# romanwerpachowski/ML

Measured on NVIDIA B200. Metric: em_point_components_per_second, higher is better.
Workload: dtype f64

## Files before the change

### ml_b200/csrc/em.cu

```cuda
#include <algorithm>
#include <cmath>
#include <limits>

#include "em_direct.cuh"
#include "em_split.cuh"
#include "fastmath.cuh"
#include "internal.h"

namespace mlb {

constexpr int kTile = 64;
constexpr int kEmThreads = 128;
constexpr int kLogBatch = 16;

__host__ __device__ constexpr int em_ne_offdiag(int DP) { return 4 * (DP / 4) * (DP / 4 - 1) / 2; }
__host__ __device__ constexpr int em_ne(int DP) { return em_ne_offdiag(DP) + 2 * (DP / 4) + (DP / 4 + 1) / 2 + DP / 4; }
__host__ __device__ constexpr int em_estep_offdiag(int DP, int a, int mb)
{
    const int DQ = DP / 4, ma = a / 4, i = a % 4;
    int n = 0;
    for (int m = 0; m < ma; ++m) n += 4 * (DQ - 1 - m);
    return n + i * (DQ - 1 - ma) + (mb - ma - 1);
}
__host__ __device__ constexpr int em_fm_raw(int DP) { return 1 + DP + DP * (DP + 1) / 2; }
__host__ __device__ constexpr int em_nm(int DP) { return (em_fm_raw(DP) + 7) / 8; }
__host__ __device__ constexpr int em_sv(int DP, int KP) { return em_nm(DP) * 8 * KP + 8; }
__host__ __device__ constexpr int em_theta_len(int DP, int KP) { return em_ne(DP) * (KP / 8) * 32 + KP; }

constexpr size_t em_smem_bytes(int DP, int KP)
{
    return sizeof(double) * (em_theta_len(DP, KP) + 2 * kTile * (DP + 4) + kTile * (KP + 4) + 8 + DP + kExpTableSize);
}

struct EmArgs {
    const double* x;
    long long n_local;
    int d, k;
    const double* shift;
    const double* theta;
    const int2* feat_m;
    double* partials;
    int chunk;
    int n_chunks;
    unsigned* counter;
    const double* r_in;
    long long r_ld;
    double* r_out;
    long long r_out_ld;
    unsigned* labels_out;
    long long range_begin, range_count;
};

__device__ __forceinline__ long long min64(long long a, long long b) { return a < b ? a : b; }

__device__ __forceinline__ void dmma(double (&acc)[2], double a, double b)
{
    asm("mma.sync.aligned.m8n8k4.row.col.f64.f64.f64.f64 {%0,%1}, {%2}, {%3}, {%0,%1};" : "+d"(acc[0]), "+d"(acc[1]) : "d"(a), "d"(b));
}

template <int NT>
__device__ __forceinline__ void load_theta_frag(const double* thE, int j, int lane, double (&bf)[NT])
{
    if constexpr (NT == 1) {
        bf[0] = thE[j * 32 + lane];
    } else {
#pragma unroll
        for (int h = 0; h < NT / 2; ++h) {
            const double2 v = reinterpret_cast<const double2*>(thE)[(j * (NT / 2) + h) * 32 + lane];
            bf[2 * h] = v.x;
            bf[2 * h + 1] = v.y;
        }
    }
}

template <int DP, int KP, int MODE>
__global__ void __launch_bounds__(kEmThreads, (DP * KP <= 128 || MODE >= 2) ? 4 : 2) em_kernel(const EmArgs p)
{
    constexpr int NT = KP / 8, DQ = DP / 4, NE = em_ne(DP), NM = em_nm(DP);
    constexpr int ZS = DP + 4, RS = KP + 4;
    constexpr int WN = (NM >= 8 || NT == 1) ? 1 : 2, WM = 4 / WN;
    constexpr int MW = (NM + WM - 1) / WM, NW = NT / WN;
    constexpr int SV = em_sv(DP, KP);
    constexpr int XR = kTile * DP / kEmThreads;

    extern __shared__ __align__(16) double sm[];
    double* thE = sm;
    double* cE = thE + NE * NT * 32;
    double* Zb = cE + KP;
    double* R = Zb + 2 * kTile * ZS;
    double* wl = R + kTile * RS;
    double* sh = wl + 8;
    double* etab = sh + DP;
    __shared__ int s_next;

    const int tid = threadIdx.x, lane = tid & 31, warp = tid >> 5, g = lane >> 2, c = lane & 3;
    const int d = p.d;

    if (MODE != 1)
        for (int i = tid; i < em_theta_len(DP, KP); i += kEmThreads) sm[i] = p.theta[i];
    for (int i = tid; i < 2 * kTile * ZS; i += kEmThreads) Zb[i] = 0.0;
    for (int i = tid; i < kTile * RS; i += kEmThreads) R[i] = 0.0;
    if (tid < DP) sh[tid] = tid < d ? p.shift[tid] : 0.0;
    load_exp_table(etab);

    const int wm = warp / WN, wn = warp % WN;
    int ia[MW], ib[MW];
    double sacc[MW][NW][2];
    if (MODE < 2) {
#pragma unroll
        for (int i = 0; i < MW; ++i) {
            const int mt = wm * MW + i;
            const int2 f = mt < NM ? p.feat_m[mt * 8 + g] : make_int2(DP + 1, DP + 1);
            ia[i] = f.x;
            ib[i] = f.y;
        }
    }

    double xr[XR];
    auto load_tile = [&](long long point0, int nvalid) {
        const double* xg = p.x + point0 * d;
        const int nel = nvalid * d;
#pragma unroll
        for (int r = 0; r < XR; ++r) {
            const int e = tid + kEmThreads * r;
            xr[r] = e < nel ? xg[e] : 0.0;
        }
    };
    auto store_tile = [&](double* Z, int nvalid) {
        const int nel = nvalid * d;
#pragma unroll
        for (int r = 0; r < XR; ++r) {
            const int e = tid + kEmThreads * r;
            if (e < kTile * d) {
                const int pt = (d == DP) ? e / DP : FastDiv(d).div(e);
                const int dm = e - pt * d;
                Z[pt * ZS + dm] = e < nel ? xr[r] - sh[dm] : 0.0;
            }
        }
        if (tid < kTile) Z[tid * ZS + DP] = tid < nvalid ? 1.0 : 0.0;
    };

    const long long work_begin = MODE >= 2 ? p.range_begin : 0;
    const long long work_end = MODE >= 2 ? p.range_begin + p.range_count : p.n_local;

    for (;;) {
        __syncthreads();
        if (tid == 0) s_next = static_cast<int>(atomicAdd(p.counter, 1u));
        __syncthreads();
        const int chunk = s_next;
        if (chunk >= p.n_chunks) break;
        const long long p_begin = work_begin + static_cast<long long>(chunk) * p.chunk;
        const long long p_end = min64(p_begin + p.chunk, work_end);
        const int ntiles = static_cast<int>((p_end - p_begin + kTile - 1) / kTile);

        if (MODE < 2) {
#pragma unroll
            for (int i = 0; i < MW; ++i)
#pragma unroll
                for (int nt = 0; nt < NW; ++nt) sacc[i][nt][0] = sacc[i][nt][1] = 0.0;
        }
        double ll_acc = 0.0, ll_prod = 1.0;

        load_tile(p_begin, static_cast<int>(min64(kTile, p_end - p_begin)));
        store_tile(Zb, static_cast<int>(min64(kTile, p_end - p_begin)));
        __syncthreads();

        for (int t = 0; t < ntiles; ++t) {
            double* Z = Zb + (t & 1) * kTile * ZS;
            const long long tile0 = p_begin + static_cast<long long>(t) * kTile;
            const int nvalid = static_cast<int>(min64(kTile, p_end - tile0));
            const int nvalid_next = t + 1 < ntiles ? static_cast<int>(min64(kTile, p_end - tile0 - kTile)) : 0;
            if (t + 1 < ntiles) load_tile(tile0 + kTile, nvalid_next);

            if (MODE == 1) {
                for (int idx = tid; idx < kTile * p.k; idx += kEmThreads) {
                    const int pt = idx % kTile, kk = idx / kTile;
                    R[pt * RS + kk] = pt < nvalid ? p.r_in[tile0 + pt + kk * p.r_ld] : 0.0;
                }
            } else {
                const double* z0 = Z + (warp * 16 + g) * ZS;
                const double* z1 = z0 + 8 * ZS;
                double acc[2][NT][2];
#pragma unroll
                for (int nt = 0; nt < NT; ++nt) {
                    const double2 cc = *reinterpret_cast<const double2*>(cE + 8 * nt + 2 * c);
                    acc[0][nt][0] = acc[1][nt][0] = cc.x;
                    acc[0][nt][1] = acc[1][nt][1] = cc.y;
                }
                double zc0[DQ], zc1[DQ];
#pragma unroll
                for (int m = 0; m < DQ; ++m) {
                    zc0[m] = z0[4 * m + c];
                    zc1[m] = z1[4 * m + c];
                }
                auto estep = [&](int j, double a0, double a1) {
                    double bf[NT];
                    load_theta_frag<NT>(thE, j, lane, bf);
#pragma unroll
                    for (int nt = 0; nt < NT; ++nt) {
                        dmma(acc[0][nt], a0, bf[nt]);
                        dmma(acc[1][nt], a1, bf[nt]);
                    }
                };
#pragma unroll
                for (int a = 0; a < DP - 4; ++a) {
                    const double za0 = z0[a], za1 = z1[a];
#pragma unroll
                    for (int m = a / 4 + 1; m < DQ; ++m) estep(em_estep_offdiag(DP, a, m), za0 * zc0[m], za1 * zc1[m]);
                }
                constexpr int J0 = em_ne_offdiag(DP);
#pragma unroll
                for (int m = 0; m < DQ; ++m) estep(J0 + m, zc0[m] * zc0[m], zc1[m] * zc1[m]);
#pragma unroll
                for (int m = 0; m < DQ; ++m) {
                    const int o = 4 * m + ((c + 1) & 3);
                    estep(J0 + DQ + m, zc0[m] * z0[o], zc1[m] * z1[o]);
                }
#pragma unroll
                for (int h = 0; h < (DQ + 1) / 2; ++h) {
                    const int mx = 2 * h + (c >> 1);
                    const int o = 4 * mx + c, o2 = 4 * mx + ((c + 2) & 3);
                    const bool live = mx < DQ;
                    const double u0 = live ? z0[o] * z0[o2] : 0.0, u1 = live ? z1[o] * z1[o2] : 0.0;
                    estep(J0 + 2 * DQ + h, u0, u1);
                }
#pragma unroll
                for (int m = 0; m < DQ; ++m) estep(NE - DQ + m, zc0[m], zc1[m]);
                double mxs[2], sums[2];
#pragma unroll
                for (int mt = 0; mt < 2; ++mt) {
                    int mkey = lse_key(acc[mt][0][0]);
#pragma unroll
                    for (int nt = 0; nt < NT; ++nt) mkey = max(mkey, max(lse_key(acc[mt][nt][0]), lse_key(acc[mt][nt][1])));
                    mkey = max(mkey, __shfl_xor_sync(0xffffffffu, mkey, 1));
                    mkey = max(mkey, __shfl_xor_sync(0xffffffffu, mkey, 2));
                    const double mx = lse_shift_of_key(mkey);
                    double sum = 0.0;
#pragma unroll
                    for (int nt = 0; nt < NT; ++nt) {
                        acc[mt][nt][0] = exp_nonpositive(acc[mt][nt][0] - mx, etab);
                        acc[mt][nt][1] = exp_nonpositive(acc[mt][nt][1] - mx, etab);
                        sum += acc[mt][nt][0] + acc[mt][nt][1];
                    }
                    sum += __shfl_xor_sync(0xffffffffu, sum, 1);
                    sum += __shfl_xor_sync(0xffffffffu, sum, 2);
                    mxs[mt] = mx;
                    sums[mt] = sum;
                }
                const double inv_mine = reciprocal_of_sum((c & 1) ? sums[1] : sums[0]);
                const double invs[2] = {__shfl_sync(0xffffffffu, inv_mine, lane & ~1), __shfl_sync(0xffffffffu, inv_mine, lane | 1)};
#pragma unroll
                for (int mt = 0; mt < 2; ++mt) {
                    const int pl = warp * 16 + mt * 8 + g;
                    const double inv = invs[mt];
                    if (c == 0 && pl < nvalid) {
                        ll_acc += mxs[mt];
                        ll_prod *= sums[mt];
                    }
                    if (MODE == 0) {
#pragma unroll
                        for (int nt = 0; nt < NT; ++nt)
                            *reinterpret_cast<double2*>(R + pl * RS + 8 * nt + 2 * c) = make_double2(acc[mt][nt][0] * inv, acc[mt][nt][1] * inv);
                    } else if (MODE == 3) {
                        if (c == 0 && pl < nvalid) p.r_out[(tile0 - p.range_begin) + pl] = (mxs[mt] + log(sums[mt])) - 0.5 * d * kLog2Pi;
                    } else {
                        double best = -1.0;
                        unsigned best_k = 0xffffffffu;
#pragma unroll
                        for (int nt = 0; nt < NT; ++nt)
#pragma unroll
                            for (int e = 0; e < 2; ++e) {
                                const int kk = 8 * nt + 2 * c + e;
                                const double r = acc[mt][nt][e] * inv;
                                if (kk < p.k) {
                                    if (pl < nvalid && p.r_out) p.r_out[(tile0 - p.range_begin) + pl + kk * p.r_out_ld] = r;
                                    if (r > best) { best = r; best_k = kk; }
                                }
                            }
#pragma unroll
                        for (int off = 1; off <= 2; off <<= 1) {
                            const double ob = __shfl_xor_sync(0xffffffffu, best, off);
                            const unsigned ok = __shfl_xor_sync(0xffffffffu, best_k, off);
                            if (ob > best || (ob == best && ok < best_k)) { best = ob; best_k = ok; }
                        }
                        if (c == 0 && pl < nvalid && p.labels_out) p.labels_out[(tile0 - p.range_begin) + pl] = best_k;
                    }
                }
            }
            if (MODE < 2) {
                __syncthreads();
#pragma unroll 4
                for (int s = 0; s < kTile / 4; ++s) {
                    const double* zp = Z + (4 * s + c) * ZS;
                    const double* rp = R + (4 * s + c) * RS + wn * NW * 8 + g;
                    double bf[NW];
#pragma unroll
                    for (int nt = 0; nt < NW; ++nt) bf[nt] = rp[8 * nt];
#pragma unroll
                    for (int i = 0; i < MW; ++i) {
                        if (wm * MW + i < NM) {
                            const double af = zp[ia[i]] * zp[ib[i]];
#pragma unroll
                            for (int nt = 0; nt < NW; ++nt) dmma(sacc[i][nt], af, bf[nt]);
                        }
                    }
                }
            }
            if (MODE != 1 && ((t & (kLogBatch - 1)) == kLogBatch - 1 || t + 1 == ntiles)) {
                ll_acc += log(ll_prod);
                ll_prod = 1.0;
            }
            if (t + 1 < ntiles) store_tile(Zb + ((t + 1) & 1) * kTile * ZS, nvalid_next);
            __syncthreads();
        }

        if (MODE < 2) {
            double* out = p.partials + static_cast<long long>(chunk) * SV;
#pragma unroll
            for (int i = 0; i < MW; ++i) {
                const int mt = wm * MW + i;
                if (mt < NM) {
#pragma unroll
                    for (int nt = 0; nt < NW; ++nt)
                        *reinterpret_cast<double2*>(out + (mt * 8 + g) * KP + (wn * NW + nt) * 8 + 2 * c) = make_double2(sacc[i][nt][0], sacc[i][nt][1]);
                }
            }
#pragma unroll
            for (int off = 16; off >= 1; off >>= 1) ll_acc += __shfl_xor_sync(0xffffffffu, ll_acc, off);
            if (lane == 0) wl[warp] = ll_acc;
            __syncthreads();
            if (tid == 0) out[NM * 8 * KP] = (wl[0] + wl[1]) + (wl[2] + wl[3]);
            if (tid >= 1 && tid < 8) out[NM * 8 * KP + tid] = 0.0;
        }
    }
}

#include "em_small.cuh"

struct EmFinalizeArgs {
    const double* vsum;
    const double* dstats;
    const double* shift;
    int d, k, DP, KP, SV;
    int DPd, dSV;
    long long n_total;
    const int2* feat_m;
    const int2* feat_e;
    int nm8, ne;
    double* means;
    double* covs;
    double* weights;
    double* inv_covs;
    double* sqrt_dets;
    double* theta_out;
    double* dimg_out;
    double* kappa_out;
    int p_in_smem;
    double* ll_ring;
    unsigned long long* ll_counter;
    int ll_ring_len;
};

__global__ void em_finalize_kernel(const EmFinalizeArgs p)
{
    extern __shared__ double fs[];
// ... 220 lines not shown
    double* ll_tile = nullptr;
    double* partials = nullptr;
    double* vsum = nullptr;
    long long* sc_begin = nullptr;
    int2* tile_tab = nullptr;
    int n_sc = 0;
    int grid_e = 0, grid_m = 0;
};

struct EmDirect {
    bool capable = false;
    bool ready = false;
    int DP = 0, NB = 0, KPr = 0, IMG = 0, L = 0, SVd = 0;
    int cb = 1, cg = 1, tiles_per_range = 0, n_ranges = 1;
    size_t smem_e = 0, smem_m = 0;
    int64_t sc_bounds[kVirtualShards + 1] = {};
    std::vector<EmDirectGpu> gpus;
    ReduceScratch scratch;
};

constexpr int kDirectMaxDim = 128;
constexpr double kKappaDirect = 3.0e5;

constexpr int kLlRing = 4096;
constexpr long long kStagePoints = 1 << 20;

}

using namespace mlb;

struct mlb_em {
    mlb_ctx* ctx = nullptr;
    mlb_data* data = nullptr;
    int d = 0, k = 0, DP = 0, KP = 0, NT = 0, NE = 0, NM = 0, SV = 0;
    std::vector<int2> feat_m, feat_e;
    std::vector<EmGpu> gpus;
    int cur = 0;
    bool have_params = false, have_step = false;
    int last_path = 0;
    int64_t direct_steps = 0;
    int64_t launches = 0;
    int64_t steps_done = 0;
    EmKernelFn fn_step = nullptr, fn_mstep = nullptr, fn_emit = nullptr, fn_score = nullptr;
    int path = 1;
    EmDirect dr;
    int forced_path = 0;
    int route = 1;
    double kappa_max = 0.0;
    bool r_direct_valid = false;
    double* kappa_host = nullptr;
    EmSplitKernelFn fn_split_e = nullptr, fn_split_m = nullptr, fn_split_score = nullptr;
    size_t smem_split_e = 0, smem_split_m = 0;
    size_t smem_fused = 0;
    int MW = 4;
    cudaGraphExec_t step_graph[2] = {nullptr, nullptr};
    int64_t launches_per_step = 0;
    int plain_steps = 0;
    ReduceScratch reduce_scratch;

    double* means(int g) const { return gpus[g].params; }
    double* covs(int g) const { return gpus[g].params + d * k; }
    double* weights(int g) const { return covs(g) + static_cast<size_t>(k) * d * d; }
    double* inv_covs(int g) const { return weights(g) + k; }
    double* sqrt_dets(int g) const { return inv_covs(g) + static_cast<size_t>(k) * d * d; }
    size_t params_len() const { return static_cast<size_t>(d) * k + 2 * static_cast<size_t>(k) * d * d + 2 * k; }
};

namespace mlb {

static int pad_to(int v, const int* options, int n)
{
    for (int i = 0; i < n; ++i)
        if (v <= options[i]) return options[i];
    return 0;
}

static EmArgs base_args(const mlb_em* em, int g)
{
    const DataShard& sh = em->data->shards[g];
    const EmGpu& eg = em->gpus[g];
    EmArgs a{};
    a.x = sh.x;
    a.n_local = sh.n();
    a.d = em->d;
    a.k = em->k;
    a.shift = sh.shift;
    a.theta = eg.theta[em->cur];
    a.feat_m = eg.feat_m;
    a.partials = eg.partials;
    a.chunk = em->data->lay.chunk;
    a.n_chunks = static_cast<int>(sh.n_chunks());
    a.counter = eg.counter;
    return a;
}

static int launch_em(mlb_em* em, EmKernelFn fn, const EmArgs& a, int g, int grid)
{
    Gpu& gpu = em->ctx->gpus[g];
    MLB_CUDA(cudaMemsetAsync(a.counter, 0, sizeof(unsigned), gpu.stream));
    if (a.n_chunks > 0) {
        const bool timed = fn == em->fn_step;
        if (timed) MLB_TRY(em->gpus[g].timer.begin(gpu.stream));
        fn<<<std::min(grid, a.n_chunks), em->DP <= 8 ? kSmallThreads : kEmThreads, em->smem_fused, gpu.stream>>>(a);
        MLB_CUDA(cudaGetLastError());
        if (timed) MLB_TRY(em->gpus[g].timer.end(gpu.stream));
        ++em->launches;
    }
    return MLB_OK;
}

static EmSplitArgs split_args(const mlb_em* em, int g, const double* theta)
{
    const DataShard& sh = em->data->shards[g];
    const EmGpu& eg = em->gpus[g];
    EmSplitArgs a{};
    a.x = sh.x;
    a.n_local = sh.n();
    a.d = em->d; a.k = em->k; a.DP = em->DP; a.KP = em->KP;
    a.shift = sh.shift;
    a.theta = theta;
    a.feat_e = eg.feat_e_off;
    a.feat_m = eg.feat_m;
    a.ne = em->NE; a.nm = em->NM;
    a.r = eg.r;
    a.partials = eg.partials;
    a.ll_tile = eg.ll_tile;
    a.sv = em->SV;
    a.chunk = em->data->lay.chunk;
    a.n_chunks = static_cast<int>(sh.n_chunks());
    a.counter = eg.counter;
    return a;
}

static int launch_split(mlb_em* em, int g, const double* theta, bool run_e, bool timed)
{
    Gpu& gpu = em->ctx->gpus[g];
    EmGpu& eg = em->gpus[g];
    const EmSplitArgs a = split_args(em, g, theta);
    if (a.n_chunks == 0) return MLB_OK;
    if (timed) MLB_TRY(eg.timer.begin(gpu.stream));
    if (run_e) {
        MLB_CUDA(cudaMemsetAsync(a.counter, 0, sizeof(unsigned), gpu.stream));
        const long long e_items = static_cast<long long>(a.n_chunks) * (a.chunk / kSpTile);
        em->fn_split_e<<<static_cast<unsigned>(std::min<long long>(eg.grid_e, e_items)), kSpThreads, em->smem_split_e, gpu.stream>>>(a);
        MLB_CUDA(cudaGetLastError());
        ++em->launches;
    }
    const int ngroups = em->KP / (em->NT * 8), nslabs = (em->NM + 4 * em->MW - 1) / (4 * em->MW);
    const long long nitems = static_cast<long long>(a.n_chunks) * nslabs * ngroups;
    MLB_REQUIRE(nitems < (1ll << 31), "EM split path: too many work items");
    MLB_CUDA(cudaMemsetAsync(a.counter, 0, sizeof(unsigned), gpu.stream));
    em->fn_split_m<<<static_cast<unsigned>(std::min<long long>(eg.grid_m, nitems)), kSpThreads, em->smem_split_m, gpu.stream>>>(a);
    MLB_CUDA(cudaGetLastError());
    ++em->launches;
    if (timed) MLB_TRY(eg.timer.end(gpu.stream));
    return MLB_OK;
// ... 505 lines not shown

extern "C" {

int mlb_selftest_exp(const double* x, int64_t n, double* out)
{
    MLB_REQUIRE(x && out && n >= 0, "mlb_selftest_exp: bad argument");
    if (n == 0) return MLB_OK;
    MLB_CUDA(cudaSetDevice(0));
    double *dx = nullptr, *dy = nullptr;
    MLB_CUDA(cudaMalloc(&dx, sizeof(double) * n));
    MLB_CUDA(cudaMalloc(&dy, sizeof(double) * n));
    MLB_CUDA(cudaMemcpy(dx, x, sizeof(double) * n, cudaMemcpyHostToDevice));
    selftest_exp_kernel<<<static_cast<unsigned>((n + 127) / 128), 128>>>(dx, n, dy);
    MLB_CUDA(cudaGetLastError());
    MLB_CUDA(cudaMemcpy(out, dy, sizeof(double) * n, cudaMemcpyDeviceToHost));
    MLB_CUDA(cudaFree(dx));
    MLB_CUDA(cudaFree(dy));
    return MLB_OK;
}

int mlb_em_create(mlb_ctx* ctx, mlb_data* data, int k, mlb_em** out)
{
    MLB_ENTER(ctx);
    MLB_REQUIRE(ctx && data && out, "mlb_em_create: null argument");
    MLB_REQUIRE(data->ctx == ctx, "mlb_em_create: data belongs to another context");
    MLB_REQUIRE(k >= 1, "mlb_em_create: number of components must be positive");
    MLB_REQUIRE(data->d <= kDirectMaxDim, "mlb_em_create: D=%d not supported by this build (D <= %d)", data->d, kDirectMaxDim);
    static const int dps[] = {4, 8, 16}, kps[] = {8, 16, 32};
    const bool fused = data->d <= 16 && k <= 32;
    const bool split = !fused && data->d <= 64 && k <= 256;
    int DP = 0, KP = 0, NT = 0;
    if (fused) {
        DP = pad_to(data->d, dps, 3);
        KP = pad_to(k, kps, 3);
        NT = KP / 8;
    } else if (split) {
        DP = (data->d + 3) / 4 * 4;
        const int KG = k > 32 ? 64 : (k > 16 ? 32 : 16);
        KP = (k + KG - 1) / KG * KG;
        NT = KG / 8;
    }
    auto* em = new mlb_em;
    em->ctx = ctx; em->data = data; em->d = data->d; em->k = k;
    em->path = fused ? 1 : split ? 2 : 0;
    em->route = em->path ? em->path : 3;
    if (em->path) {
        em->DP = DP; em->KP = KP; em->NT = NT; em->NE = em_ne(DP); em->NM = em_nm(DP); em->SV = em_sv(DP, KP);
    }
    if (fused) {
        em->fn_step = em_kernel_for<0>(DP, KP);
        em->fn_mstep = em_kernel_for<1>(DP, KP);
        em->fn_emit = em_kernel_for<2>(DP, KP);
        em->fn_score = em_kernel_for<3>(DP, KP);
        em->smem_fused = DP <= 8 ? em_small_smem_bytes(DP, KP) : em_smem_bytes(DP, KP);
    } else if (split) {
        em->fn_split_e = NT == 8 ? em_split_e_kernel<8> : NT == 4 ? em_split_e_kernel<4> : em_split_e_kernel<2>;
        em->fn_split_score = NT == 8 ? em_split_e_kernel<8 + kSpScore> : NT == 4 ? em_split_e_kernel<4 + kSpScore> : em_split_e_kernel<2 + kSpScore>;
        int best_waste = 1 << 30;
        for (int mw = 3; mw <= 5; ++mw) {
            const int slabs = (em->NM + 4 * mw - 1) / (4 * mw), waste = slabs * 4 * mw - em->NM;
            if (waste <= best_waste) { best_waste = waste; em->MW = mw; }
        }
        if (NT == 8) em->fn_split_m = em->MW == 3 ? em_split_m_kernel<8, 3> : em->MW == 4 ? em_split_m_kernel<8, 4> : em_split_m_kernel<8, 5>;
        else if (NT == 4) em->fn_split_m = em->MW == 3 ? em_split_m_kernel<4, 3> : em->MW == 4 ? em_split_m_kernel<4, 4> : em_split_m_kernel<4, 5>;
        else em->fn_split_m = em->MW == 3 ? em_split_m_kernel<2, 3> : em->MW == 4 ? em_split_m_kernel<2, 4> : em_split_m_kernel<2, 5>;
        em->smem_split_e = em_split_e_smem(NT, DP, KP);
        em->smem_split_m = em_split_m_smem(NT, DP);
    }
    if (em->path) {
        em->feat_e.assign(static_cast<size_t>(em->NE) * 4, make_int2(-1, -1));
        const int DQ = DP / 4, J0 = em_ne_offdiag(DP);
        auto put = [&](int j, int c, int a, int b) { em->feat_e[static_cast<size_t>(j) * 4 + c] = make_int2(std::min(a, b), std::max(a, b)); };
        for (int a = 0; a < DP - 4; ++a)
            for (int m = a / 4 + 1; m < DQ; ++m)
                for (int c = 0; c < 4; ++c) put(em_estep_offdiag(DP, a, m), c, a, 4 * m + c);
        for (int m = 0; m < DQ; ++m)
            for (int c = 0; c < 4; ++c) {
                put(J0 + m, c, 4 * m + c, 4 * m + c);
                put(J0 + DQ + m, c, 4 * m + c, 4 * m + ((c + 1) & 3));
            }
        for (int h = 0; h < (DQ + 1) / 2; ++h)
            for (int c = 0; c < 4; ++c) {
                const int mx = 2 * h + (c >> 1);
                if (mx < DQ) put(J0 + 2 * DQ + h, c, 4 * mx + c, 4 * mx + ((c + 2) & 3));
            }
        for (int m = 0; m < DQ; ++m)
            for (int c = 0; c < 4; ++c) em->feat_e[static_cast<size_t>(em->NE - DQ + m) * 4 + c] = make_int2(4 * m + c, DP);
        em->feat_m.assign(static_cast<size_t>(em->NM) * 8, make_int2(DP + 1, DP + 1));
        size_t f = 0;
        em->feat_m[f++] = make_int2(DP, DP);
        for (int a = 0; a < DP; ++a) em->feat_m[f++] = make_int2(a, DP);
        for (int a = 0; a < DP; ++a)
            for (int b = a; b < DP; ++b) em->feat_m[f++] = make_int2(a, b);
    }
    if (fused && DP <= 8) {
        for (size_t f = 0; f < em->feat_m.size(); ++f) {
            int2 ab = make_int2(DP + 1, DP + 1);
            if (f < em->feat_e.size() && em->feat_e[f].x >= 0) ab = em->feat_e[f];
            if (static_cast<int>(f) == em_small_count_slot(DP)) ab = make_int2(DP, DP);
            em->feat_m[f] = ab;
        }
    }
    {
        EmDirect& dr = em->dr;
        dr.capable = true;
        dr.DP = (em->d + 7) / 8 * 8;
        dr.NB = dr.DP / 8;
        dr.KPr = (k + 7) / 8 * 8;
        dr.IMG = dr_img_len(dr.DP);
        dr.L = dr_stat_len(dr.DP);
        const long long svd = static_cast<long long>(k) * dr.L + 8;
        if (svd >= (1ll << 31)) { delete em; set_error("mlb_em_create: D=%d, K=%d: statistics vector too long", data->d, k); return MLB_EINVAL; }
        dr.SVd = static_cast<int>(svd);
        dr.cb = static_cast<int>(std::max<size_t>(1, std::min<size_t>(std::min(16, k), (12 * 1024) / (sizeof(double) * dr.IMG))));
        const int T = dr_tiles(dr.NB);
        if (T <= 4 * kDrSlots) {
            const int by_smem = static_cast<int>((96 * 1024) / (sizeof(double) * 2 * kDrSub * (dr.DP + 12))) - 1;
            dr.cg = std::max(1, std::min({16, k, 4 * kDrSlots / T, by_smem}));
            dr.tiles_per_range = T;
            dr.n_ranges = 1;
        } else {
            dr.cg = 1;
            dr.tiles_per_range = 4 * kDrSlots;
            dr.n_ranges = (T + 4 * kDrSlots - 1) / (4 * kDrSlots);
        }
        dr.smem_e = em_direct_e_smem(dr.DP, dr.cb);
        dr.smem_m = em_direct_m_smem(dr.DP, dr.cg, em->d);
        dr.sc_bounds[0] = 0;
        for (int v = 0; v < kVirtualShards; ++v)
            dr.sc_bounds[v + 1] = dr.sc_bounds[v] + std::min<int64_t>(data->lay.vshard_chunk[v + 1] - data->lay.vshard_chunk[v], kDrSuperPerVshard);
        dr.gpus.resize(ctx->gpus.size());
    }
    em->gpus.resize(ctx->gpus.size());
    int rc = for_each_gpu(ctx, [&](int g, Gpu& gpu) -> int {
        EmGpu& eg = em->gpus[g];
        EmDirectGpu& dg = em->dr.gpus[g];
        const DataShard& sh = data->shards[g];
        MLB_CUDA(cudaMallocFromPoolAsync(&eg.params, sizeof(double) * em->params_len(), gpu.pool, gpu.stream));
        MLB_CUDA(cudaMallocFromPoolAsync(&eg.ll, sizeof(double) * kLlRing, gpu.pool, gpu.stream));
        MLB_CUDA(cudaMallocFromPoolAsync(&eg.ll_counter, sizeof(unsigned long long), gpu.pool, gpu.stream));
        MLB_CUDA(cudaMemsetAsync(eg.ll_counter, 0, sizeof(unsigned long long), gpu.stream));
        MLB_CUDA(cudaMallocFromPoolAsync(&eg.counter, sizeof(unsigned), gpu.pool, gpu.stream));
        MLB_CUDA(cudaMallocFromPoolAsync(&dg.img, sizeof(double) * static_cast<size_t>(k) * em->dr.IMG, gpu.pool, gpu.stream));
        MLB_CUDA(cudaMallocFromPoolAsync(&dg.kappa, sizeof(double) * k, gpu.pool, gpu.stream));
        MLB_CUDA(cudaMemsetAsync(dg.kappa, 0, sizeof(double) * k, gpu.stream));
        {
            const size_t fin_smem = finalize_smem(em, nullptr);
            if (fin_smem > 48 * 1024)
                MLB_CUDA(cudaFuncSetAttribute(reinterpret_cast<const void*>(em_finalize_kernel), cudaFuncAttributeMaxDynamicSharedMemorySize, static_cast<int>(fin_smem)));
        }
        int sms = 0;
        MLB_CUDA(cudaDeviceGetAttribute(&sms, cudaDevAttrMultiProcessorCount, gpu.device));
        if (em->path) {
            const size_t theta_len = static_cast<size_t>(em_theta_len(DP, KP));
            MLB_CUDA(cudaMallocFromPoolAsync(&eg.theta[0], sizeof(double) * theta_len, gpu.pool, gpu.stream));
            MLB_CUDA(cudaMallocFromPoolAsync(&eg.theta[1], sizeof(double) * theta_len, gpu.pool, gpu.stream));
            MLB_CUDA(cudaMallocFromPoolAsync(&eg.partials, sizeof(double) * std::max<int64_t>(1, sh.n_chunks()) * em->SV, gpu.pool, gpu.stream));
            MLB_CUDA(cudaMallocFromPoolAsync(&eg.vsum, sizeof(double) * kVirtualShards * em->SV, gpu.pool, gpu.stream));
            MLB_CUDA(cudaMallocFromPoolAsync(&eg.feat_m, sizeof(int2) * em->feat_m.size(), gpu.pool, gpu.stream));
            MLB_CUDA(cudaMallocFromPoolAsync(&eg.feat_e, sizeof(int2) * em->feat_e.size(), gpu.pool, gpu.stream));
            MLB_CUDA(cudaMemsetAsync(eg.vsum, 0, sizeof(double) * kVirtualShards * em->SV, gpu.stream));
            MLB_CUDA(cudaMemcpyAsync(eg.feat_m, em->feat_m.data(), sizeof(int2) * em->feat_m.size(), cudaMemcpyHostToDevice, gpu.stream));
            MLB_CUDA(cudaMemcpyAsync(eg.feat_e, em->feat_e.data(), sizeof(int2) * em->feat_e.size(), cudaMemcpyHostToDevice, gpu.stream));
        }
        if (em->path == 1) {
            const size_t smem = em->smem_fused;
            for (EmKernelFn fn : {em->fn_step, em->fn_mstep, em->fn_emit, em->fn_score})
                MLB_CUDA(cudaFuncSetAttribute(reinterpret_cast<const void*>(fn), cudaFuncAttributeMaxDynamicSharedMemorySize, static_cast<int>(smem)));
            int per_sm = 0;
            MLB_CUDA(cudaOccupancyMaxActiveBlocksPerMultiprocessor(&per_sm, reinterpret_cast<const void*>(em->fn_step), em->DP <= 8 ? kSmallThreads : kEmThreads, smem));
            MLB_REQUIRE(per_sm >= 1, "mlb_em_create: EM kernel does not fit on an SM");
            eg.grid = per_sm * sms;
        } else if (em->path == 2) {
            std::vector<int2> off(em->feat_e.size());
            for (size_t i = 0; i < off.size(); ++i) off[i] = em->feat_e[i].x < 0 ? make_int2(DP + 1, DP + 1) : em->feat_e[i];
            MLB_CUDA(cudaMallocFromPoolAsync(&eg.feat_e_off, sizeof(int2) * off.size(), gpu.pool, gpu.stream));
            MLB_CUDA(cudaMemcpyAsync(eg.feat_e_off, off.data(), sizeof(int2) * off.size(), cudaMemcpyHostToDevice, gpu.stream));
            MLB_CUDA(cudaStreamSynchronize(gpu.stream));
            MLB_CUDA(cudaMallocFromPoolAsync(&eg.r, sizeof(double) * std::max<int64_t>(1, sh.n()) * KP, gpu.pool, gpu.stream));
            {
                const size_t n_tiles = static_cast<size_t>(std::max<int64_t>(1, sh.n_chunks())) * (data->lay.chunk / kSpTile);
                MLB_CUDA(cudaMallocFromPoolAsync(&eg.ll_tile, sizeof(double) * n_tiles, gpu.pool, gpu.stream));
                MLB_CUDA(cudaMemsetAsync(eg.ll_tile, 0, sizeof(double) * n_tiles, gpu.stream));
            }
            MLB_CUDA(cudaMemsetAsync(eg.partials, 0, sizeof(double) * std::max<int64_t>(1, sh.n_chunks()) * em->SV, gpu.stream));
            MLB_CUDA(cudaFuncSetAttribute(reinterpret_cast<const void*>(em->fn_split_e), cudaFuncAttributeMaxDynamicSharedMemorySize, static_cast<int>(em->smem_split_e)));
            MLB_CUDA(cudaFuncSetAttribute(reinterpret_cast<const void*>(em->fn_split_score), cudaFuncAttributeMaxDynamicSharedMemorySize, static_cast<int>(em->smem_split_e)));
            MLB_CUDA(cudaFuncSetAttribute(reinterpret_cast<const void*>(em->fn_split_m), cudaFuncAttributeMaxDynamicSharedMemorySize, static_cast<int>(em->smem_split_m)));
            int per_e = 0, per_m = 0;
            MLB_CUDA(cudaOccupancyMaxActiveBlocksPerMultiprocessor(&per_e, reinterpret_cast<const void*>(em->fn_split_e), kSpThreads, em->smem_split_e));
            MLB_CUDA(cudaOccupancyMaxActiveBlocksPerMultiprocessor(&per_m, reinterpret_cast<const void*>(em->fn_split_m), kSpThreads, em->smem_split_m));
            MLB_REQUIRE(per_e >= 1 && per_m >= 1, "mlb_em_create: EM kernels do not fit on an SM (D=%d, K=%d)", em->d, em->k);
            eg.grid_e = per_e * sms;
            eg.grid_m = per_m * sms;
        }
        MLB_CUDA(cudaStreamSynchronize(gpu.stream));
        return MLB_OK;
    });
    if (rc != MLB_OK) { mlb_em_destroy(em); return rc; }
    *out = em;
    return MLB_OK;
}

int mlb_em_destroy(mlb_em* em)
{
    MLB_ENTER(em ? em->ctx : nullptr);
    if (!em) return MLB_OK;
    for (cudaGraphExec_t& ge : em->step_graph)
        if (ge) { cudaGraphExecDestroy(ge); ge = nullptr; }
    for (size_t g = 0; g < em->gpus.size(); ++g) {
        cudaSetDevice(em->ctx->gpus[g].device);
        cudaStreamSynchronize(em->ctx->gpus[g].stream);
        EmGpu& eg = em->gpus[g];
        eg.timer.destroy();
        for (void* ptr : {static_cast<void*>(eg.theta[0]), static_cast<void*>(eg.theta[1]), static_cast<void*>(eg.params),
                          static_cast<void*>(eg.partials), static_cast<void*>(eg.vsum), static_cast<void*>(eg.ll), static_cast<void*>(eg.ll_counter),
                          static_cast<void*>(eg.feat_m), static_cast<void*>(eg.feat_e), static_cast<void*>(eg.counter),
                          static_cast<void*>(eg.stage), static_cast<void*>(eg.stage_labels), static_cast<void*>(eg.r), static_cast<void*>(eg.ll_tile),
                          static_cast<void*>(eg.feat_e_off)})
            if (ptr) cudaFreeAsync(ptr, em->ctx->gpus[g].stream);
        if (g < em->dr.gpus.size()) {
// ... 76 lines not shown
}

int mlb_em_conditioning(mlb_em* em, double* kappa_max, int* next_path)
{
    MLB_ENTER(em ? em->ctx : nullptr);
    MLB_REQUIRE(em, "mlb_em_conditioning: null argument");
    if (kappa_max) *kappa_max = em->kappa_max;
    if (next_path) *next_path = em->route;
    return MLB_OK;
}

int mlb_em_get_params(mlb_em* em, double* means, double* covariances, double* weights)
{
    MLB_ENTER(em ? em->ctx : nullptr);
    MLB_REQUIRE(em, "mlb_em_get_params: null argument");
    if (!em->have_params) { set_error("mlb_em_get_params: parameters not set"); return MLB_ESTATE; }
    Gpu& gpu = em->ctx->gpus[0];
    MLB_CUDA(cudaSetDevice(gpu.device));
    if (means) MLB_CUDA(cudaMemcpyAsync(means, em->means(0), sizeof(double) * em->d * em->k, cudaMemcpyDeviceToHost, gpu.stream));
    if (covariances) MLB_CUDA(cudaMemcpyAsync(covariances, em->covs(0), sizeof(double) * em->k * em->d * em->d, cudaMemcpyDeviceToHost, gpu.stream));
    if (weights) MLB_CUDA(cudaMemcpyAsync(weights, em->weights(0), sizeof(double) * em->k, cudaMemcpyDeviceToHost, gpu.stream));
    MLB_CUDA(cudaStreamSynchronize(gpu.stream));
    return MLB_OK;
}

int mlb_em_get_precisions(mlb_em* em, double* inverse_covariances, double* sqrt_determinants)
{
    MLB_ENTER(em ? em->ctx : nullptr);
    MLB_REQUIRE(em, "mlb_em_get_precisions: null argument");
    if (!em->have_params) { set_error("mlb_em_get_precisions: parameters not set"); return MLB_ESTATE; }
    Gpu& gpu = em->ctx->gpus[0];
    MLB_CUDA(cudaSetDevice(gpu.device));
    if (inverse_covariances)
        MLB_CUDA(cudaMemcpyAsync(inverse_covariances, em->inv_covs(0), sizeof(double) * em->k * em->d * em->d, cudaMemcpyDeviceToHost, gpu.stream));
    if (sqrt_determinants) MLB_CUDA(cudaMemcpyAsync(sqrt_determinants, em->sqrt_dets(0), sizeof(double) * em->k, cudaMemcpyDeviceToHost, gpu.stream));
    MLB_CUDA(cudaStreamSynchronize(gpu.stream));
    return MLB_OK;
}

int mlb_em_sample_covariance(mlb_em* em, double* cov_out)
{
    MLB_ENTER(em ? em->ctx : nullptr);
    MLB_REQUIRE(em && cov_out, "mlb_em_sample_covariance: null argument");
    if (em->path == 0 || em->forced_path == 3) return direct_sample_covariance(em, cov_out);
    const int d = em->d, DP = em->DP;
    const bool narrow = em->path == 1 && em->KP > 8;
    const int KP = narrow ? 8 : em->KP, SV = narrow ? em_sv(DP, 8) : em->SV;
    std::vector<double> theta(em_theta_len(DP, KP), 0.0);
    for (int kk = 1; kk < KP; ++kk) theta[static_cast<size_t>(em->NE) * (KP / 8) * 32 + kk] = -std::numeric_limits<double>::infinity();
    MLB_TRY(for_each_gpu(em->ctx, [&](int g, Gpu& gpu) -> int {
        MLB_CUDA(cudaMemcpyAsync(em->gpus[g].theta[em->cur ^ 1], theta.data(), sizeof(double) * theta.size(), cudaMemcpyHostToDevice, gpu.stream));
        if (!narrow) return launch_pass(em, g, em->gpus[g].theta[em->cur ^ 1], false);
        const EmKernelFn fn = em_kernel_for<0>(DP, 8);
        const size_t smem = DP <= 8 ? em_small_smem_bytes(DP, 8) : em_smem_bytes(DP, 8);
        MLB_CUDA(cudaFuncSetAttribute(reinterpret_cast<const void*>(fn), cudaFuncAttributeMaxDynamicSharedMemorySize, static_cast<int>(smem)));
        int per_sm = 0, sms = 0;
        MLB_CUDA(cudaOccupancyMaxActiveBlocksPerMultiprocessor(&per_sm, reinterpret_cast<const void*>(fn), em->DP <= 8 ? kSmallThreads : kEmThreads, smem));
        MLB_CUDA(cudaDeviceGetAttribute(&sms, cudaDevAttrMultiProcessorCount, gpu.device));
        MLB_REQUIRE(per_sm >= 1, "mlb_em_sample_covariance: kernel does not fit on an SM");
        EmArgs a = base_args(em, g);
        a.theta = em->gpus[g].theta[em->cur ^ 1];
        a.k = 1;
        MLB_CUDA(cudaMemsetAsync(a.counter, 0, sizeof(unsigned), gpu.stream));
        if (a.n_chunks > 0) {
            fn<<<std::min(per_sm * sms, a.n_chunks), em->DP <= 8 ? kSmallThreads : kEmThreads, smem, gpu.stream>>>(a);
            MLB_CUDA(cudaGetLastError());
            ++em->launches;
        }
        return MLB_OK;
    }));
    if (em->path == 2) em->have_step = false;
    std::vector<double*> partials, vsum;
    for (EmGpu& eg : em->gpus) { partials.push_back(eg.partials); vsum.push_back(eg.vsum); }
    MLB_TRY(reduce_and_exchange(em->data, partials, vsum, SV, em->reduce_scratch));
    em->launches += static_cast<int64_t>(em->ctx->gpus.size());
    std::vector<double> host(static_cast<size_t>(kVirtualShards) * SV);
    Gpu& gpu0 = em->ctx->gpus[0];
    MLB_CUDA(cudaSetDevice(gpu0.device));
    MLB_CUDA(cudaMemcpyAsync(host.data(), em->gpus[0].vsum, sizeof(double) * host.size(), cudaMemcpyDeviceToHost, gpu0.stream));
    MLB_TRY(mlb_ctx_synchronize(em->ctx));
    double count = 0;
    std::vector<double> m1(d, 0.0), m2(static_cast<size_t>(d) * d, 0.0);
    for (size_t f = 0; f < em->feat_m.size(); ++f) {
        const int2 ab = em->feat_m[f];
        const double val = tree8(host.data() + f * KP, SV);
        if (ab.x == DP && ab.y == DP) count = val;
        else if (ab.y == DP && ab.x < d) m1[ab.x] = val;
        else if (ab.x < d && ab.y < d) { m2[ab.x + static_cast<size_t>(ab.y) * d] = val; m2[ab.y + static_cast<size_t>(ab.x) * d] = val; }
    }
    for (int a = 0; a < d; ++a)
        for (int b = 0; b < d; ++b)
            cov_out[a + static_cast<size_t>(b) * d] = (m2[a + static_cast<size_t>(b) * d] - m1[a] * m1[b] / count) / (count - 1.0);
    return MLB_OK;
}

int mlb_em_mstep_from_responsibilities(mlb_em* em, const double* resp, int64_t ld)
{
    MLB_ENTER(em ? em->ctx : nullptr);
    MLB_REQUIRE(em && resp, "mlb_em_mstep_from_responsibilities: null argument");
    mlb_ctx* ctx = em->ctx;
    const int64_t host_begin = ctx->rank_mode ? em->data->shards[0].begin : 0;
    std::vector<double*> dev(ctx->gpus.size(), nullptr);
    const int rc = for_each_gpu(ctx, [&](int g, Gpu& gpu) -> int {
        const DataShard& sh = em->data->shards[g];
        const int64_t n = std::max<int64_t>(1, sh.n());
        MLB_CUDA(cudaMallocFromPoolAsync(&dev[g], sizeof(double) * n * em->k, gpu.pool, gpu.stream));
        if (sh.n() > 0)
// ... 381 lines not shown
```

Before: 48.58.

## Stage pairwise feature products in shared memory and halve fused-step tile

The fused E+M kernel (modes 0/1) now uses a 32-point tile and writes the E-step's quadratic feature values into a shared-memory feature table. The M-step accumulation reads those precomputed products directly instead of recomputing z[a]*z[b] from gathered indices held in registers. The table stride is padded to avoid bank conflicts, and emit/score kernels keep the 64-point tile with their own shared-memory size. This frees the index registers and removes a multiply and gather per MMA operand. In exchange it adds shared-memory writes in the E-step, extra shared memory, and more per-tile sync overhead from the smaller tile.

```diff
diff --git a/ml_b200/csrc/em.cu b/ml_b200/csrc/em.cu
--- a/ml_b200/csrc/em.cu
+++ b/ml_b200/csrc/em.cu
@@ -27,9 +27,14 @@
 __host__ __device__ constexpr int em_sv(int DP, int KP) { return em_nm(DP) * 8 * KP + 8; }
 __host__ __device__ constexpr int em_theta_len(int DP, int KP) { return em_ne(DP) * (KP / 8) * 32 + KP; }
 
-constexpr size_t em_smem_bytes(int DP, int KP)
-{
-    return sizeof(double) * (em_theta_len(DP, KP) + 2 * kTile * (DP + 4) + kTile * (KP + 4) + 8 + DP + kExpTableSize);
+__host__ __device__ constexpr int em_tile(int MODE) { return MODE < 2 ? 32 : kTile; }
+__host__ __device__ constexpr int em_table_stride(int DP) { return em_nm(DP) * 8 + 4; }
+
+constexpr size_t em_smem_bytes(int DP, int KP, int MODE)
+{
+    const int tile = em_tile(MODE);
+    return sizeof(double) * (em_theta_len(DP, KP) + 2 * tile * (DP + 4) + tile * (KP + 4) + (MODE < 2 ? tile * em_table_stride(DP) : 0) + 8 + DP +
+                             kExpTableSize);
 }
 
 struct EmArgs {
@@ -77,18 +82,25 @@
 __global__ void __launch_bounds__(kEmThreads, (DP * KP <= 128 || MODE >= 2) ? 4 : 2) em_kernel(const EmArgs p)
 {
     constexpr int NT = KP / 8, DQ = DP / 4, NE = em_ne(DP), NM = em_nm(DP);
-    constexpr int ZS = DP + 4, RS = KP + 4;
+    constexpr int ZS = DP + 4, RS = KP + 4, TS = em_table_stride(DP);
     constexpr int WN = (NM >= 8 || NT == 1) ? 1 : 2, WM = 4 / WN;
     constexpr int MW = (NM + WM - 1) / WM, NW = NT / WN;
     constexpr int SV = em_sv(DP, KP);
-    constexpr int XR = kTile * DP / kEmThreads;
+    constexpr int TILE = em_tile(MODE), MT = TILE / 32, PW = 8 * MT;
+    constexpr int XR = TILE * DP / kEmThreads;
+    constexpr int LB = kLogBatch * 2 / MT;
+    constexpr int CNT = NE * 4;
+    static_assert(TS % 8 == 4, "feature table stride: bank-conflict-free only at 4 mod 8 doubles");
+    static_assert(DQ % 2 == 0 && CNT < NM * 8, "the count row follows the last E-step slot (em_small_count_slot)");
+    static_assert(MODE != 0 || MT == 1, "the E-step fills the feature table from one m-tile per warp");
 
     extern __shared__ __align__(16) double sm[];
     double* thE = sm;
     double* cE = thE + NE * NT * 32;
     double* Zb = cE + KP;
-    double* R = Zb + 2 * kTile * ZS;
-    double* wl = R + kTile * RS;
+    double* R = Zb + 2 * TILE * ZS;
+    double* T = R + TILE * RS;
+    double* wl = T + (MODE < 2 ? TILE * TS : 0);
     double* sh = wl + 8;
     double* etab = sh + DP;
     __shared__ int s_next;
@@ -98,23 +110,15 @@
 
     if (MODE != 1)
         for (int i = tid; i < em_theta_len(DP, KP); i += kEmThreads) sm[i] = p.theta[i];
-    for (int i = tid; i < 2 * kTile * ZS; i += kEmThreads) Zb[i] = 0.0;
-    for (int i = tid; i < kTile * RS; i += kEmThreads) R[i] = 0.0;
+    for (int i = tid; i < 2 * TILE * ZS; i += kEmThreads) Zb[i] = 0.0;
+    for (int i = tid; i < TILE * RS; i += kEmThreads) R[i] = 0.0;
+    if (MODE < 2)
+        for (int i = tid; i < TILE * TS; i += kEmThreads) T[i] = 0.0;
     if (tid < DP) sh[tid] = tid < d ? p.shift[tid] : 0.0;
     load_exp_table(etab);
 
     const int wm = warp / WN, wn = warp % WN;
-    int ia[MW], ib[MW];
     double sacc[MW][NW][2];
-    if (MODE < 2) {
-#pragma unroll
-        for (int i = 0; i < MW; ++i) {
-            const int mt = wm * MW + i;
-            const int2 f = mt < NM ? p.feat_m[mt * 8 + g] : make_int2(DP + 1, DP + 1);
-            ia[i] = f.x;
-            ib[i] = f.y;
-        }
-    }
 
     double xr[XR];
     auto load_tile = [&](long long point0, int nvalid) {
@@ -131,13 +135,13 @@
 #pragma unroll
         for (int r = 0; r < XR; ++r) {
             const int e = tid + kEmThreads * r;
-            if (e < kTile * d) {
+            if (e < TILE * d) {
                 const int pt = (d == DP) ? e / DP : FastDiv(d).div(e);
                 const int dm = e - pt * d;
                 Z[pt * ZS + dm] = e < nel ? xr[r] - sh[dm] : 0.0;
             }
         }
-        if (tid < kTile) Z[tid * ZS + DP] = tid < nvalid ? 1.0 : 0.0;
+        if (tid < TILE) Z[tid * ZS + DP] = tid < nvalid ? 1.0 : 0.0;
     };
 
     const long long work_begin = MODE >= 2 ? p.range_begin : 0;
@@ -151,7 +155,7 @@
         if (chunk >= p.n_chunks) break;
         const long long p_begin = work_begin + static_cast<long long>(chunk) * p.chunk;
         const long long p_end = min64(p_begin + p.chunk, work_end);
-        const int ntiles = static_cast<int>((p_end - p_begin + kTile - 1) / kTile);
+        const int ntiles = static_cast<int>((p_end - p_begin + TILE - 1) / TILE);
 
         if (MODE < 2) {
 #pragma unroll
@@ -161,31 +165,36 @@
         }
         double ll_acc = 0.0, ll_prod = 1.0;
 
-        load_tile(p_begin, static_cast<int>(min64(kTile, p_end - p_begin)));
-        store_tile(Zb, static_cast<int>(min64(kTile, p_end - p_begin)));
+        load_tile(p_begin, static_cast<int>(min64(TILE, p_end - p_begin)));
+        store_tile(Zb, static_cast<int>(min64(TILE, p_end - p_begin)));
         __syncthreads();
 
         for (int t = 0; t < ntiles; ++t) {
-            double* Z = Zb + (t & 1) * kTile * ZS;
-            const long long tile0 = p_begin + static_cast<long long>(t) * kTile;
-            const int nvalid = static_cast<int>(min64(kTile, p_end - tile0));
-            const int nvalid_next = t + 1 < ntiles ? static_cast<int>(min64(kTile, p_end - tile0 - kTile)) : 0;
-            if (t + 1 < ntiles) load_tile(tile0 + kTile, nvalid_next);
+            double* Z = Zb + (t & 1) * TILE * ZS;
+            const long long tile0 = p_begin + static_cast<long long>(t) * TILE;
+            const int nvalid = static_cast<int>(min64(TILE, p_end - tile0));
+            const int nvalid_next = t + 1 < ntiles ? static_cast<int>(min64(TILE, p_end - tile0 - TILE)) : 0;
+            if (t + 1 < ntiles) load_tile(tile0 + TILE, nvalid_next);
 
             if (MODE == 1) {
-                for (int idx = tid; idx < kTile * p.k; idx += kEmThreads) {
-                    const int pt = idx % kTile, kk = idx / kTile;
+                for (int idx = tid; idx < TILE * p.k; idx += kEmThreads) {
+                    const int pt = idx % TILE, kk = idx / TILE;
                     R[pt * RS + kk] = pt < nvalid ? p.r_in[tile0 + pt + kk * p.r_ld] : 0.0;
                 }
+                for (int f = tid; f < NM * 8; f += kEmThreads) {
+                    const int2 ab = p.feat_m[f];
+#pragma unroll 4
+                    for (int pt = 0; pt < TILE; ++pt) T[pt * TS + f] = Z[pt * ZS + ab.x] * Z[pt * ZS + ab.y];
+                }
             } else {
-                const double* z0 = Z + (warp * 16 + g) * ZS;
+                const double* z0 = Z + (warp * PW + g) * ZS;
                 const double* z1 = z0 + 8 * ZS;
-                double acc[2][NT][2];
+                double acc[MT][NT][2];
 #pragma unroll
                 for (int nt = 0; nt < NT; ++nt) {
                     const double2 cc = *reinterpret_cast<const double2*>(cE + 8 * nt + 2 * c);
-                    acc[0][nt][0] = acc[1][nt][0] = cc.x;
-                    acc[0][nt][1] = acc[1][nt][1] = cc.y;
+                    acc[0][nt][0] = acc[MT - 1][nt][0] = cc.x;
+                    acc[0][nt][1] = acc[MT - 1][nt][1] = cc.y;
                 }
                 double zc0[DQ], zc1[DQ];
 #pragma unroll
@@ -193,13 +202,15 @@
                     zc0[m] = z0[4 * m + c];
                     zc1[m] = z1[4 * m + c];
                 }
+                double* tw = T + (warp * PW + g) * TS + c;
                 auto estep = [&](int j, double a0, double a1) {
+                    if constexpr (MODE == 0) tw[4 * j] = a0;
                     double bf[NT];
                     load_theta_frag<NT>(thE, j, lane, bf);
 #pragma unroll
                     for (int nt = 0; nt < NT; ++nt) {
                         dmma(acc[0][nt], a0, bf[nt]);
-                        dmma(acc[1][nt], a1, bf[nt]);
+                        if constexpr (MT == 2) dmma(acc[1][nt], a1, bf[nt]);
                     }
                 };
 #pragma unroll
@@ -226,9 +237,10 @@
                 }
 #pragma unroll
                 for (int m = 0; m < DQ; ++m) estep(NE - DQ + m, zc0[m], zc1[m]);
-                double mxs[2], sums[2];
-#pragma unroll
-                for (int mt = 0; mt < 2; ++mt) {
+                if (MODE == 0 && c == 0) tw[CNT] = warp * PW + g < nvalid ? 1.0 : 0.0;
+                double mxs[MT], sums[MT];
+#pragma unroll
+                for (int mt = 0; mt < MT; ++mt) {
                     int mkey = lse_key(acc[mt][0][0]);
 #pragma unroll
                     for (int nt = 0; nt < NT; ++nt) mkey = max(mkey, max(lse_key(acc[mt][nt][0]), lse_key(acc[mt][nt][1])));
@@ -247,11 +259,12 @@
                     mxs[mt] = mx;
                     sums[mt] = sum;
                 }
-                const double inv_mine = reciprocal_of_sum((c & 1) ? sums[1] : sums[0]);
-                const double invs[2] = {__shfl_sync(0xffffffffu, inv_mine, lane & ~1), __shfl_sync(0xffffffffu, inv_mine, lane | 1)};
-#pragma unroll
-                for (int mt = 0; mt < 2; ++mt) {
-                    const int pl = warp * 16 + mt * 8 + g;
+                const double inv_mine = reciprocal_of_sum((c & 1) ? sums[MT - 1] : sums[0]);
+                const double invs[2] = {MT == 2 ? __shfl_sync(0xffffffffu, inv_mine, lane & ~1) : inv_mine,
+                                        MT == 2 ? __shfl_sync(0xffffffffu, inv_mine, lane | 1) : inv_mine};
+#pragma unroll
+                for (int mt = 0; mt < MT; ++mt) {
+                    const int pl = warp * PW + mt * 8 + g;
                     const double inv = invs[mt];
                     if (c == 0 && pl < nvalid) {
                         ll_acc += mxs[mt];
@@ -290,8 +303,8 @@
             if (MODE < 2) {
                 __syncthreads();
 #pragma unroll 4
-                for (int s = 0; s < kTile / 4; ++s) {
-                    const double* zp = Z + (4 * s + c) * ZS;
+                for (int s = 0; s < TILE / 4; ++s) {
+                    const double* tp = T + (4 * s + c) * TS + wm * MW * 8 + g;
                     const double* rp = R + (4 * s + c) * RS + wn * NW * 8 + g;
                     double bf[NW];
 #pragma unroll
@@ -299,18 +312,18 @@
 #pragma unroll
                     for (int i = 0; i < MW; ++i) {
                         if (wm * MW + i < NM) {
-                            const double af = zp[ia[i]] * zp[ib[i]];
+                            const double af = tp[8 * i];
 #pragma unroll
                             for (int nt = 0; nt < NW; ++nt) dmma(sacc[i][nt], af, bf[nt]);
                         }
                     }
                 }
             }
-            if (MODE != 1 && ((t & (kLogBatch - 1)) == kLogBatch - 1 || t + 1 == ntiles)) {
+            if (MODE != 1 && ((t & (LB - 1)) == LB - 1 || t + 1 == ntiles)) {
                 ll_acc += log(ll_prod);
                 ll_prod = 1.0;
             }
-            if (t + 1 < ntiles) store_tile(Zb + ((t + 1) & 1) * kTile * ZS, nvalid_next);
+            if (t + 1 < ntiles) store_tile(Zb + ((t + 1) & 1) * TILE * ZS, nvalid_next);
             __syncthreads();
         }
 
@@ -637,6 +650,7 @@
     EmSplitKernelFn fn_split_e = nullptr, fn_split_m = nullptr, fn_split_score = nullptr;
     size_t smem_split_e = 0, smem_split_m = 0;
     size_t smem_fused = 0;
+    size_t smem_fused_e = 0;
     int MW = 4;
     cudaGraphExec_t step_graph[2] = {nullptr, nullptr};
     int64_t launches_per_step = 0;
@@ -686,7 +700,8 @@
     if (a.n_chunks > 0) {
         const bool timed = fn == em->fn_step;
         if (timed) MLB_TRY(em->gpus[g].timer.begin(gpu.stream));
-        fn<<<std::min(grid, a.n_chunks), em->DP <= 8 ? kSmallThreads : kEmThreads, em->smem_fused, gpu.stream>>>(a);
+        const size_t smem = fn == em->fn_emit || fn == em->fn_score ? em->smem_fused_e : em->smem_fused;
+        fn<<<std::min(grid, a.n_chunks), em->DP <= 8 ? kSmallThreads : kEmThreads, smem, gpu.stream>>>(a);
         MLB_CUDA(cudaGetLastError());
         if (timed) MLB_TRY(em->gpus[g].timer.end(gpu.stream));
         ++em->launches;
@@ -1298,7 +1313,8 @@
         em->fn_mstep = em_kernel_for<1>(DP, KP);
         em->fn_emit = em_kernel_for<2>(DP, KP);
         em->fn_score = em_kernel_for<3>(DP, KP);
-        em->smem_fused = DP <= 8 ? em_small_smem_bytes(DP, KP) : em_smem_bytes(DP, KP);
+        em->smem_fused = DP <= 8 ? em_small_smem_bytes(DP, KP) : em_smem_bytes(DP, KP, 0);
+        em->smem_fused_e = DP <= 8 ? em_small_smem_bytes(DP, KP) : em_smem_bytes(DP, KP, 2);
     } else if (split) {
         em->fn_split_e = NT == 8 ? em_split_e_kernel<8> : NT == 4 ? em_split_e_kernel<4> : em_split_e_kernel<2>;
         em->fn_split_score = NT == 8 ? em_split_e_kernel<8 + kSpScore> : NT == 4 ? em_split_e_kernel<4 + kSpScore> : em_split_e_kernel<2 + kSpScore>;
@@ -1339,7 +1355,7 @@
         for (int a = 0; a < DP; ++a)
             for (int b = a; b < DP; ++b) em->feat_m[f++] = make_int2(a, b);
     }
-    if (fused && DP <= 8) {
+    if (fused) {
         for (size_t f = 0; f < em->feat_m.size(); ++f) {
             int2 ab = make_int2(DP + 1, DP + 1);
             if (f < em->feat_e.size() && em->feat_e[f].x >= 0) ab = em->feat_e[f];
@@ -1411,8 +1427,10 @@
         }
         if (em->path == 1) {
             const size_t smem = em->smem_fused;
-            for (EmKernelFn fn : {em->fn_step, em->fn_mstep, em->fn_emit, em->fn_score})
+            for (EmKernelFn fn : {em->fn_step, em->fn_mstep})
                 MLB_CUDA(cudaFuncSetAttribute(reinterpret_cast<const void*>(fn), cudaFuncAttributeMaxDynamicSharedMemorySize, static_cast<int>(smem)));
+            for (EmKernelFn fn : {em->fn_emit, em->fn_score})
+                MLB_CUDA(cudaFuncSetAttribute(reinterpret_cast<const void*>(fn), cudaFuncAttributeMaxDynamicSharedMemorySize, static_cast<int>(em->smem_fused_e)));
             int per_sm = 0;
             MLB_CUDA(cudaOccupancyMaxActiveBlocksPerMultiprocessor(&per_sm, reinterpret_cast<const void*>(em->fn_step), em->DP <= 8 ? kSmallThreads : kEmThreads, smem));
             MLB_REQUIRE(per_sm >= 1, "mlb_em_create: EM kernel does not fit on an SM");
@@ -1595,7 +1613,7 @@
         MLB_CUDA(cudaMemcpyAsync(em->gpus[g].theta[em->cur ^ 1], theta.data(), sizeof(double) * theta.size(), cudaMemcpyHostToDevice, gpu.stream));
         if (!narrow) return launch_pass(em, g, em->gpus[g].theta[em->cur ^ 1], false);
         const EmKernelFn fn = em_kernel_for<0>(DP, 8);
-        const size_t smem = DP <= 8 ? em_small_smem_bytes(DP, 8) : em_smem_bytes(DP, 8);
+        const size_t smem = DP <= 8 ? em_small_smem_bytes(DP, 8) : em_smem_bytes(DP, 8, 0);
         MLB_CUDA(cudaFuncSetAttribute(reinterpret_cast<const void*>(fn), cudaFuncAttributeMaxDynamicSharedMemorySize, static_cast<int>(smem)));
         int per_sm = 0, sms = 0;
         MLB_CUDA(cudaOccupancyMaxActiveBlocksPerMultiprocessor(&per_sm, reinterpret_cast<const void*>(fn), em->DP <= 8 ? kSmallThreads : kEmThreads, smem));
```

After: 48.99 (median of 6 runs). No clear change (+0.9%).
